# ThorLL/Element-Crush-Gym

Hardware: AMD Instinct MI355X
Metric: env-steps/sec (batched boards) at 1/2/4/8 MI355X, 9×9×6; bit-exact vs CPU (higher is better)
Workload: dtype int8; 1 GPU; C3: 1,048,576 boards per GPU, 9x9x6, Match3Env.step x 7466 (step kernel + overflow fixup + autoreset; N>1: RCCL reward/done all-gather once after the last step); boards_per_gpu=1048576, num_moves=20, env_goal=500, parallelism=dp1, hw_queues=8, autoreset=True

## Files before the change

### element-crush-gym_amd/csrc/m3_api.hip

```cpp
#include "m3_kernels.hpp"

#include <string>

namespace {
thread_local std::string g_err;
}

int set_err(int code, const char* fmt, ...) {
    char buf[512];
    va_list ap;
    va_start(ap, fmt);
    vsnprintf(buf, sizeof(buf), fmt, ap);
    va_end(ap);
    g_err = buf;
    return code;
}

#ifdef M3_SPLIT_TU
namespace m3k {
M3_INSTANTIATE(extern template, CF_0)
M3_INSTANTIATE(extern template, CF_1)
#ifndef M3_HEADLINE_ONLY
M3_INSTANTIATE(extern template, CF_2)
M3_INSTANTIATE(extern template, CF_3)
// ... 600 lines not shown
    return cnt[2] ? bad_cells_error() : M3_OK;
}

int m3_env_create(m3_ctx* c, int64_t n, int num_moves, int env_goal, m3_env** out) {
    CHECK_ARG(c && out && n > 0 && num_moves > 0, "bad arguments");
    CHECK_ARG(n < (int64_t)1 << 31, "n too large");
    int rc0 = check_ids_on_board(c);
    if (rc0) return rc0;
    *out = nullptr;
    HIP_TRY(hipSetDevice(c->device));
    m3_env* e = new m3_env;
    e->ctx = c;
    e->n = n;
    e->num_moves = num_moves;
    e->goal = env_goal;
    const size_t bytes = n * (size_t)c->N;
    hipError_t err = hipSuccess;
    auto alloc = [&](auto** p, size_t sz) {
        if (err == hipSuccess) err = hipMalloc((void**)p, sz ? sz : 4);
    };
    alloc(&e->boards[0], bytes);
    alloc(&e->boards[1], bytes);
    alloc(&e->seeds, n * 4);
    alloc(&e->flags, n * 4);
    alloc(&e->draws, n * 4);
    alloc(&e->legal, n * 4ull * c->AW);
    alloc(&e->score, n * 4);
    alloc(&e->moves, n * 4);
    alloc(&e->next_action, n * 4);
    alloc(&e->reward, n * 4);
    alloc(&e->done, n);
    alloc(&e->trunc, n);
    alloc(&e->counters, 64 * 4 * MAX_SHARDS);
    alloc(&e->ovf_list, n * 4);
    alloc(&e->packed, 2 * n * 4);
    alloc(&e->slot, n);
    alloc(&e->ne_words, (size_t)NSLOT * n * 4ull * ((c->N + 3) / 4));
    alloc(&e->ne_first, (size_t)NSLOT * n * 4);
    alloc(&e->ne_legal, (size_t)NSLOT * n * 4ull * c->AW);
    alloc(&e->ne_flags, (size_t)NSLOT * n * 4);
    alloc(&e->defer, n * 4);
    for (int p = 0; p < PF_LAG; ++p) {
        alloc(&e->pf_list[p], n * 4);
        alloc(&e->pf_seed[p], n * 4);
        alloc(&e->pf_slot[p], n * 4);
    }
    with_shape(c->shape, [&](auto cf) {
        using K = KS<decltype(cf)>;
        using St = LdsStore<decltype(cf), K::GCAP, K::B>;
        alloc(&e->spill, (size_t)MAX_SHARDS * K::SPILL_RECORDS * St::SPILL_WORDS * 4);
        alloc(&e->m397, (size_t)NSLOT * n * 4ull);
        constexpr size_t RW = CONT_REC<decltype(cf)>;
        if constexpr (K::CASCADE_LIMIT >= 0) alloc(&e->cont, RW * n * 4ull);
        if constexpr (RESET_TWO_STAGE<decltype(cf)>) alloc(&e->tab, (size_t)TwoStage<decltype(cf)>::TW * n * 4ull);
        if constexpr (RESET_TWO_STAGE_REJ<decltype(cf)>)
            alloc(&e->tab, (size_t)TwoStageRej<decltype(cf)>::TW * n * 4ull);
        return 0;
    });
    for (hipEvent_t& ev : e->gev)
        if (err == hipSuccess) err = hipEventCreateWithFlags(&ev, hipEventDisableTiming);
    {
        void* zp[] = {e->boards[0], e->boards[1], e->seeds, e->flags, e->draws, e->legal, e->score, e->moves,
                      e->next_action, e->reward, e->done, e->trunc, e->slot};
        size_t zb[] = {bytes, bytes, n * 4ull, n * 4ull, n * 4ull, n * 4ull * c->AW, n * 4ull, n * 4ull,
                       n * 4ull, n * 4ull, (size_t)n, (size_t)n, (size_t)n};
        for (int i = 0; i < 13 && err == hipSuccess; ++i) err = hipMemset(zp[i], 0, zb[i]);
    }
    if (err != hipSuccess) {
        m3_env_destroy(e);
        return set_err(M3_ERR_HIP, "env allocation (%lld boards): %s", (long long)n, hipGetErrorString(err));
    }
    int rc = m3_env_set_shards(e, 1);
    if (rc) {
        m3_env_destroy(e);
        return rc;
    }
    *out = e;
    return M3_OK;
}

int m3_env_set_shards(m3_env* e, int nshards) {
    CHECK_ARG(e && nshards >= 1 && nshards <= MAX_SHARDS, "nshards must be in [1, 8]");
    HIP_TRY(hipSetDevice(e->ctx->device));
    int rc = sync_env(e);
    if (rc) return rc;
    destroy_shards(e);
    const int64_t per = ((e->n + nshards - 1) / nshards + BLOCK - 1) / BLOCK * BLOCK;
    for (int s = 0; s < nshards; ++s) {
        m3_env::Shard sh;
        sh.off = std::min<int64_t>(e->n, s * per);
        sh.n = std::min<int64_t>(e->n, sh.off + per) - sh.off;
        if (M3_STREAM_PRIO) {
            int least = 0, greatest = 0;
            HIP_TRY(hipDeviceGetStreamPriorityRange(&least, &greatest));
            HIP_TRY(hipStreamCreateWithPriority(&sh.stream, hipStreamNonBlocking, greatest));
            HIP_TRY(hipStreamCreateWithPriority(&sh.pstream, hipStreamNonBlocking, least));
        } else {
            HIP_TRY(hipStreamCreateWithFlags(&sh.stream, hipStreamNonBlocking));
            HIP_TRY(hipStreamCreateWithFlags(&sh.pstream, hipStreamNonBlocking));
        }
        HIP_TRY(hipEventCreateWithFlags(&sh.ev, hipEventDisableTiming));
        for (hipEvent_t& ev : sh.pev) HIP_TRY(hipEventCreateWithFlags(&ev, hipEventDisableTiming));
        for (hipEvent_t& ev : sh.aev) HIP_TRY(hipEventCreateWithFlags(&ev, hipEventDisableTiming));
        e->shards.push_back(sh);
    }
    return M3_OK;
}

int m3_env_synchronize(m3_env* e) {
    CHECK_ARG(e, "null env");
    HIP_TRY(hipSetDevice(e->ctx->device));
    int rc = sync_env(e);
    if (rc) return rc;
    return ensure_fresh(e);
}

int m3_env_destroy(m3_env* e) {
    if (!e) return M3_OK;
    (void)hipSetDevice(e->ctx->device);
    (void)sync_env(e);
    destroy_shards(e);
    for (int p = 0; p < 2; ++p) {
        if (e->upload_ev[p]) (void)hipEventDestroy(e->upload_ev[p]);
        if (e->hstage[p]) (void)hipHostFree(e->hstage[p]);
    }
    if (e->ustream) (void)hipStreamDestroy(e->ustream);
    for (hipEvent_t ev : e->gev)
        if (ev) (void)hipEventDestroy(ev);
    void* ptrs[] = {e->boards[0], e->boards[1], e->seeds, e->flags, e->draws, e->legal, e->score, e->moves,
                    e->next_action, e->reward, e->done, e->trunc, e->actions[0], e->actions[1], e->counters,
                    e->ovf_list,
                    e->packed, e->gathered, e->slot, e->ne_words, e->ne_first, e->ne_legal, e->ne_flags,
                    e->spill, e->m397, e->cont, e->defer, e->tab};
    for (void* p : ptrs)
        if (p) (void)hipFree(p);
    for (int q = 0; q < PF_LAG; ++q)
        for (void* p : {(void*)e->pf_list[q], (void*)e->pf_seed[q], (void*)e->pf_slot[q]})
            if (p) (void)hipFree(p);
    if (e->comm) ncclCommDestroy(e->comm);
    for (hipEvent_t ev : e->tev) (void)hipEventDestroy(ev);
    delete e;
    return M3_OK;
}

int m3_env_reset(m3_env* e, const uint32_t* seeds, uint32_t seed_base) {
    CHECK_ARG(e, "null env");
    m3_ctx* c = e->ctx;
    HIP_TRY(hipSetDevice(c->device));
    int rc0 = sync_env(e);
    if (rc0) return rc0;
    if (seeds) {
        HIP_TRY(hipMemcpyAsync(e->seeds, seeds, e->n * 4, hipMemcpyHostToDevice, c->stream));
    } else {
        uint32_t* h = (uint32_t*)malloc(e->n * 4);
        if (!h) return set_err(M3_ERR_INVALID, "host allocation failed");
        for (int64_t i = 0; i < e->n; ++i) h[i] = seed_base + (uint32_t)i;
        hipError_t err = hipMemcpy(e->seeds, h, e->n * 4, hipMemcpyHostToDevice);
        free(h);
        HIP_TRY(err);
    }
    InitArgs a{};
    a.shape = c->sdesc;
    a.n = e->n;
    a.seeds = e->seeds;
    a.boards = e->boards[e->cur];
    a.first_action = e->next_action;
    a.legal = e->legal;
    a.score = e->score;
    a.moves = e->moves;
    a.reward = e->reward;
    a.done = e->done;
    a.trunc = e->trunc;
    a.flags = e->flags;
    a.draws = e->draws;
    a.m397 = e->m397;
    a.cstride = e->n;
    HIP_TRY(hipMemsetAsync(e->counters, 0, 64 * 4 * MAX_SHARDS, c->stream));
    HIP_TRY(hipMemsetAsync(e->slot, 0, e->n, c->stream));
    e->steps = 0;
    int rc = with_shape(c->shape, [&](auto cf) {
        int r = launch_init<decltype(cf)>(c->stream, a, e->n);
        if (r == M3_OK && e->autoreset) r = fill_next_slots<decltype(cf)>(e);
        return r;
    });
    if (rc) return rc;
    HIP_TRY(hipStreamSynchronize(c->stream));
// ... 338 lines not shown
```

### element-crush-gym_amd/csrc/m3_kernels.hpp

```cpp
#pragma once
#include <hip/hip_runtime.h>
#include <rccl/rccl.h>

#include <stdarg.h>
#include <stdio.h>
#include <string.h>

#include <algorithm>
#include <string>
#include <vector>

#include "../../include/m3.h"
#include "m3_rules.hpp"

using namespace m3;

int set_err(int code, const char* fmt, ...) __attribute__((format(printf, 2, 3)));

namespace {


#define HIP_TRY(expr)                                                                            \
    do {                                                                                         \
        hipError_t e_ = (expr);                                                                  \
        if (e_ != hipSuccess)                                                                    \
            return set_err(M3_ERR_HIP, "%s: %s (%s:%d)", #expr, hipGetErrorString(e_), __FILE__, \
                           __LINE__);                                                            \
    } while (0)

#define RCCL_TRY(expr)                                                                            \
    do {                                                                                          \
        ncclResult_t r_ = (expr);                                                                 \
        if (r_ != ncclSuccess) return set_err(M3_ERR_RCCL, "%s: %s", #expr, ncclGetErrorString(r_)); \
    } while (0)

#define CHECK_ARG(cond, msg)                                       \
    do {                                                           \
        if (!(cond)) return set_err(M3_ERR_INVALID, "%s", (msg)); \
    } while (0)

constexpr int BLOCK = 256;
constexpr int FIX_BLOCK = 64;
constexpr int FIX_GRID = 16;
constexpr int INIT_FIX_BLOCK = 64;
constexpr int INIT_BLOCK = 64;
#ifndef M3_WIDE_FRAME_LANES
#define M3_WIDE_FRAME_LANES 1
#endif
template <class CF>
constexpr uint32_t lanes_for() { return CF::W > 8 ? (uint32_t)M3_WIDE_FRAME_LANES : 64u; }
template <class CF>
constexpr bool INIT_INLINE_FIX = CF::N <= 128;
constexpr int MAX_SHARDS = 8;
#ifndef M3_RESET_KCAP
#define M3_RESET_KCAP 454
#endif
constexpr uint32_t RESET_KCAP = M3_RESET_KCAP;
#ifndef M3_PF_DIV
#define M3_PF_DIV 1
#endif
#ifndef M3_PF_DIV16
#define M3_PF_DIV16 2
#endif
#ifndef M3_COOP_GMAX
#define M3_COOP_GMAX 4096
#endif
#ifndef M3_PF_GRID
#define M3_PF_GRID 0
#endif
#ifndef M3_PF_COOP_GRID
#define M3_PF_COOP_GRID 0
#endif
#ifndef M3_RESET16_CHAIN2
#define M3_RESET16_CHAIN2 0
#endif
constexpr uint32_t RESET_ROUND_CAP = 1u << 14;

template <class CF>
struct KS {
    static constexpr int B = 64;
    static_assert(B == 64, "one-wave workgroups: lds_sync() orders a single wave's LDS accesses");
    static constexpr int GCAP = CF::N <= 128 ? 6 : 4;
    static constexpr int BPW = CF::W > 8 ? M3_WIDE_FRAME_LANES : B;
#ifndef M3_STEP_WPS
#define M3_STEP_WPS 4
#endif
#ifndef M3_STEP_WPS16
#define M3_STEP_WPS16 2
#endif
#ifndef M3_STEP_WPS_FRAME
#define M3_STEP_WPS_FRAME 1
#endif
    static constexpr int STEP_WPS = CF::DYN ? M3_STEP_WPS_FRAME : (CF::N > 128 ? M3_STEP_WPS16 : M3_STEP_WPS);
#ifndef M3_CONT_WPS
#define M3_CONT_WPS M3_STEP_WPS
#endif
    static constexpr int CONT_WPS = CF::N > 128 ? 1 : M3_CONT_WPS;
    static constexpr uint32_t SPILL_RECORDS = CF::W > 8 ? 256 : 4096;
    using Chain = std::conditional_t<(CF::N > 128), ChainMT1, ChainMT>;
    using Rng = Chain;
#ifndef M3_STEP_PRIO
#define M3_STEP_PRIO 0
#endif
#ifndef M3_STREAM_PRIO
#define M3_STREAM_PRIO 0
#endif
#ifndef M3_CASCADE_LIMIT
#define M3_CASCADE_LIMIT 2
#endif
#ifndef M3_CASCADE_LIMIT16
#define M3_CASCADE_LIMIT16 -1
#endif
    static constexpr int CASCADE_LIMIT = CF::N > 128 ? M3_CASCADE_LIMIT16 : M3_CASCADE_LIMIT;
};

#ifdef __HIP_DEVICE_COMPILE__
#define M3_LDS_AS __attribute__((address_space(3)))
#else
// ... 385 lines not shown
        ArrayStore<CF> st;
        apply_and_emit<CF>(P, a, b, mt, st, dm);
        planes_to_bytes<CF>(P, reinterpret_cast<uint8_t*>(a.out_boards + b * dm.cells()), dm);
    }
    if (a.clear_ovf) {
        __syncthreads();
        if (threadIdx.x == 0) *a.ovf_count = 0u;
    }
}

#ifndef M3_NSLOT
#define M3_NSLOT 4
#endif
constexpr int NSLOT = M3_NSLOT;
static_assert(NSLOT >= 2 && NSLOT <= 255, "slot index is a byte");
constexpr int PF_LAG = NSLOT - 1;
constexpr int CBLOCKS = PF_LAG + 1;
static_assert(8 * CBLOCKS <= 40, "the counter blocks end where a shard's stats begin (m3_env::counters, word 40)");
#ifndef M3_STAGE_PAD
#define M3_STAGE_PAD 1
#endif

}
namespace m3k {
struct InitArgs {
    Shape shape;
    int64_t n;
    const uint32_t* list;
    const uint32_t* list_seed;
    const uint32_t* list_slot;
    const uint32_t* list_count;
    const uint32_t* seeds;
    uint32_t seed_add;
    uint32_t slot0;
    const uint8_t* slot_of;
    int64_t sstride;
    int8_t* boards;
    uint32_t* board_words;
    uint32_t* draws;
    int32_t* first_action;
    uint32_t* legal;
    int32_t* score;
    int32_t* moves;
    int32_t* reward;
    uint8_t* done;
    uint8_t* trunc;
    uint32_t* flags;
    uint32_t* slot_flags;
    uint32_t* stats;
    uint32_t* m397;
    int64_t cstride;
    uint32_t* defer;
    uint32_t* defer_count;
    uint32_t* tab;
};
}
using m3k::InitArgs;
namespace {

__device__ __forceinline__ void init_item(const InitArgs& a, int64_t i, int64_t& b, uint32_t& seed, uint32_t& slot) {
    if (a.list) {
        b = (int64_t)a.list[i];
        seed = a.list_seed[i];
        slot = a.list_slot[i];
    } else {
        b = i;
        seed = a.seeds[b] + a.seed_add;
        slot = a.slot_of ? ((uint32_t)a.slot_of[b] + a.slot0) % (uint32_t)NSLOT : a.slot0;
    }
}

template <class CF>
__device__ __forceinline__ void init_store_board(const InitArgs& a, int64_t ob, const typename CF::Bd* P,
                                                 const typename CF::Dim& dm) {
    if constexpr (CF::DYN) {
        uint8_t* dst = a.board_words ? reinterpret_cast<uint8_t*>(a.board_words + ob * cell_words<CF>(dm))
                                     : reinterpret_cast<uint8_t*>(a.boards + ob * dm.cells());
        frame_to_bytes<CF>(P, dst, dm);
        return;
    }
    constexpr int NW = (CF::N + 3) / 4;
    uint32_t cw[NW];
    words_from_planes<CF>(P, cw);
    if (a.board_words) {
#pragma unroll
        for (int q = 0; q < NW; ++q) a.board_words[ob * NW + q] = cw[q];
    } else {
        store_cells<CF::N>(reinterpret_cast<uint8_t*>(a.boards + ob * CF::N), cw);
    }
}

template <class CF>
__device__ __forceinline__ void init_outputs(const InitArgs& a, int64_t b, int64_t ob, uint32_t seed, uint32_t m397,
                                             uint32_t draws, const typename CF::Bd* P,
                                             const typename CF::Dim& dm = typename CF::Dim{}) {
    typename CF::Bd HL, VL;
    legal_masks<CF>(P, special_mask<CF, CF::NP>(P), HL, VL, dm);
    uint32_t act[CF::AW];
    action_bits<CF>(HL, VL, act, dm);
    ChainMT rng;
    rng.init(seed, m397);
    const int fa = random_action<CF>(act, rng);
    if (a.draws) a.draws[ob] = draws;
    if (a.first_action) a.first_action[ob] = fa;
    if (a.legal) store_legal<CF>(a.legal + ob * dm.aw(), act, dm);
    if (a.score) a.score[b] = 0;
// ... 94 lines not shown
    uint32_t x = __builtin_amdgcn_readfirstlane(seed);
    for (int blk = 0; blk < 9; ++blk) {
        uint32_t col = 0u;
#pragma unroll
        for (int j = 0; j < 64; ++j) {
            asm volatile("v_writelane_b32 %0, %1, %2" : "+v"(col) : "s"(x), "n"(j));
            x = mt_init_next(x, (uint32_t)(blk * 64 + j) + 1u);
        }
        key[blk * 64 + lane] = col;
    }
    uint32_t col = 0u;
#pragma unroll
    for (int j = 0; j < 48; ++j) {
        asm volatile("v_writelane_b32 %0, %1, %2" : "+v"(col) : "s"(x), "n"(j));
        x = mt_init_next(x, (uint32_t)(576 + j) + 1u);
    }
    if (lane < 48) key[576 + lane] = col;
}

template <class CF>
__device__ uint32_t wave_reset(const InitArgs& a, int64_t item, uint32_t* key, uint8_t* cells, int lane) {
    int64_t b;
    uint32_t seed, slot;
    init_item(a, item, b, seed, slot);
    wave_init_key(key, seed, lane);
    wave_sync();
    const uint32_t m397 = key[397];
    uint32_t pos = 624u, k = 0u;
    typename CF::Bd P[CF::NP], mask;
    const int64_t ob = (int64_t)slot * a.sstride + b;
    constexpr int NW = (CF::N + 3) / 4;
    wave_fill<CF>(key, cells, lane, pos, k, nullptr);
    planes_from_words<CF>(reinterpret_cast<const uint32_t*>(cells), P);
    while (get_match_mask<CF>(P, mask)) {
        wave_fill<CF>(key, cells, lane, pos, k, &mask);
        planes_from_words<CF>(reinterpret_cast<const uint32_t*>(cells), P);
    }
    if (a.m397 && lane == 0) a.m397[(int64_t)slot * a.cstride + b] = m397;
    if (lane == 0) init_outputs<CF>(a, b, ob, seed, m397, k, P);
    if (a.board_words) {
        for (int q = lane; q < NW; q += 64)
            a.board_words[ob * NW + q] = reinterpret_cast<const uint32_t*>(cells)[q];
    } else {
        int8_t* dst = a.boards + ob * CF::N;
        for (int x = lane; x < CF::N; x += 64) dst[x] = (int8_t)cells[x];
    }
    wave_sync();
    return k;
}

template <class CF, bool REDO>
__global__ void __launch_bounds__(INIT_BLOCK) k_init(InitArgs a) {
    const int64_t cnt = a.list_count ? (int64_t)*a.list_count : a.n;
    if (a.stats && blockIdx.x == 0 && threadIdx.x == 0) atomicAdd(&a.stats[0], (uint32_t)cnt);
    __shared__ uint32_t tm_s[CF::BITS * TileGen<CF>::TWMAX * INIT_BLOCK];
    __shared__ uint32_t pos_s[TileGen<CF>::MAXR * INIT_BLOCK];
    uint32_t* tm = tm_s + threadIdx.x;
    uint32_t* pos = pos_s + threadIdx.x;
#ifdef M3_PHASE_PROF
    M3_PROF_LDS(INIT_BLOCK)
    Prof<NoStore> ps;
    ps.w = prof_s[threadIdx.x >> 6];
    const bool live = (int64_t)blockIdx.x * INIT_BLOCK < cnt;
    if (live) ps.begin();
#else
    NoStore* const pp = nullptr;
#endif
    static_assert(INIT_INLINE_FIX<CF> && INIT_BLOCK == 64, "the in-wave redo is one wave's");
    __shared__ uint32_t key_s[REDO ? 624 : 1];
    __shared__ __attribute__((aligned(16))) uint8_t cell_s[REDO ? (CF::N + 3) / 4 * 4 + 16 : 16];
    for (int64_t base = (int64_t)blockIdx.x * INIT_BLOCK; base < cnt; base += (int64_t)gridDim.x * INIT_BLOCK) {
        const int64_t i = base + threadIdx.x;
        bool ok = true;
        if (i < cnt) {
            int64_t b;
            uint32_t seed, slot;
            init_item(a, i, b, seed, slot);
            const uint32_t m397 = mt_state397(seed);
            const uint32_t kcap = a.defer ? RESET_KCAP : 624u;
#ifdef M3_PHASE_PROF
            ok = init_emit<CF>(a, b, seed, slot, m397, tm, pos, &ps, kcap);
#else
            ok = init_emit<CF>(a, b, seed, slot, m397, tm, pos, pp, kcap);
#endif
        }
        uint64_t bad = __ballot(!ok);
        if (!REDO) {
            if (bad) {
                const int lane = (int)threadIdx.x;
                uint32_t base = 0;
                if (lane == 0) base = atomicAdd(a.defer_count, (uint32_t)__popcll(bad));
                base = __shfl(base, 0);
                if (!ok) a.defer[base + (uint32_t)__popcll(bad & ((1ull << lane) - 1ull))] = (uint32_t)i;
            }
            continue;
        }
        if (bad && a.stats && threadIdx.x == 0) atomicAdd(&a.stats[1], (uint32_t)__builtin_popcountll(bad));
        if constexpr (REDO) {
            while (bad) {
                const int l = __builtin_ctzll(bad);
                bad &= bad - 1ull;
                wave_reset<CF>(a, __shfl(i, l), key_s, cell_s, (int)threadIdx.x);
            }
        }
    }
#ifdef M3_PHASE_PROF
    if (live) ps.end(1);
#endif
}

template <class CF>
__global__ void __launch_bounds__(64) k_init_coop(InitArgs a) {
    __shared__ uint32_t key_s[624];
    __shared__ __attribute__((aligned(16))) uint8_t cell_s[(CF::N + 3) / 4 * 4 + 16];
    const uint32_t cnt = *a.defer_count;
    const int lane = (int)threadIdx.x;
    for (uint32_t q = blockIdx.x; q < cnt; q += gridDim.x) {
        wave_reset<CF>(a, a.defer[q], key_s, cell_s, lane);
        if (a.stats && lane == 0) atomicAdd(&a.stats[1], 1u);
    }
}

template <class R, class = void>
struct HasBulk : std::false_type {};
template <class R>
struct HasBulk<R, std::void_t<decltype(std::declval<R&>().bulk_ready(1u))>> : std::true_type {};

template <class CF, class RNG>
__device__ __forceinline__ void fill_round(typename CF::Bd* P, RNG& mt, const typename CF::Bd* only) {
#pragma unroll
    for (int w = 0; w < CF::W; ++w) {
        constexpr int BITS = CF::BITS;
        const int nbits = CF::N - 32 * w < 32 ? CF::N - 32 * w : 32;
        uint32_t t[BITS];
#pragma unroll
        for (int p = 0; p < BITS; ++p) t[p] = 0u;
        int bit = 0;
        if constexpr (CF::TILE_RNG != 0u && CF::TILE_RNG == CF::TILE_MASK && HasBulk<RNG>::value) {
            if (mt.bulk_ready((uint32_t)nbits)) {
#pragma unroll
                for (int j = 0; j < nbits; ++j) {
                    const uint32_t v = (mt.bulk_out((uint32_t)j) & CF::TILE_MASK) + 1u;
#pragma unroll
                    for (int p = 0; p < BITS; ++p) t[p] |= ((v >> p) & 1u) << j;
                }
                mt.bulk_skip((uint32_t)nbits);
                bit = nbits;
            }
        }
        for (; bit < nbits; ++bit) {
            uint32_t v = 1u;
            if constexpr (CF::TILE_RNG != 0u) {
                do {
                    v = mt.next32() & CF::TILE_MASK;
                } while (v > CF::TILE_RNG);
                v += 1u;
            }
#pragma unroll
            for (int p = 0; p < BITS; ++p) t[p] |= ((v >> p) & 1u) << bit;
        }
        const uint32_t m = only ? only->w[w] : 0xFFFFFFFFu;
#pragma unroll
        for (int p = 0; p < BITS; ++p) P[p].w[w] = (P[p].w[w] & ~m) | (t[p] & m);
    }
}
// ... 385 lines not shown
        lds_to_planes<CF>(lds, t, P, dm);
        legal_masks<CF>(P, special_mask<CF, CF::NP>(P), HL, VL, dm);
        uint32_t act[CF::AW];
        action_bits<CF>(HL, VL, act, dm);
        store_legal<CF>(legal + (b0 + t) * dm.aw(), act, dm);
    }
}


}
namespace m3k {
struct EnvArgs {
    Shape shape;
    int64_t n;
    int num_moves, goal;
    int autoreset;
    uint32_t stride;
    const int8_t* cur;
    int8_t* nxt;
    const int32_t* actions;
    uint32_t* seeds;
    int32_t* score;
    int32_t* moves;
    int32_t* next_action;
    int32_t* reward;
    uint8_t* done;
    uint8_t* trunc;
    uint32_t* flags;
    uint32_t* draws;
    uint32_t* legal;
    int32_t* packed;
    uint32_t* counters;
    uint32_t* spill;
    uint32_t* stats;
    uint32_t* ovf_list;
    uint8_t* slot;
    const uint32_t* ne_words;
    const int32_t* ne_first;
    const uint32_t* ne_legal;
    const uint32_t* ne_flags;
    uint32_t* pf_list;
    uint32_t* pf_seed;
    uint32_t* pf_slot;
    const uint32_t* m397;
    int64_t cstride;
    uint32_t* cont;
    int64_t cont_stride;
    uint32_t* zero_next;
};
}
using m3k::EnvArgs;
namespace {

enum : int { CNT_OVF = 0, CNT_PF_DEFER = 2, CNT_SPILL = 3, CNT_CONT = 4, CNT_PF = 5 };

template <class CF>
struct EnvFin {
    static constexpr bool CELLS_IN_REGS = !CF::DYN;
    static constexpr int NWS = (CF::N + 3) / 4;
    uint32_t ndraws, f, nflags, s_old, seed;
    int r, tr, dn, sc, mv1, na, first;
    bool reset;
    int64_t ob;
    uint32_t act[CF::AW];
    uint32_t lg[CF::AW];
    uint32_t cw[CELLS_IN_REGS ? NWS : 1];
};

template <class CF, class RNG, class Store>
__device__ __forceinline__ bool env_fin_begin(typename CF::Bd* P, const EnvArgs& a, int64_t b, RNG& rng, Store& st,
                                              int r, uint32_t f, const typename CF::Bd& HL, const typename CF::Bd& VL,
                                              int mv, int sc0, const typename CF::Dim& dm, uint8_t* row,
                                              EnvFin<CF>& e, const uint32_t* known_slot = nullptr,
                                              const uint32_t* known_seed = nullptr, bool cells = true) {
    const bool stepped = !(f & (FLAG_TERMINAL | FLAG_BAD_ACTION));
    e.r = r;
    e.sc = sc0 + r;
    e.mv1 = mv + 1;
    e.tr = e.sc >= a.goal;
    e.dn = e.tr || e.mv1 == a.num_moves;
    e.ndraws = stepped ? rng.draws() : 0u;
    action_bits<CF>(HL, VL, e.act, dm);
    e.na = -1;
    if (stepped) {
        e.na = random_action<CF>(e.act, rng);
        if (rng.overflow) return false;
        if (e.na < 0) f |= FLAG_NO_LEGAL;
    }
    e.f = f;
    mark<PH_NEXT>(st);
    e.reset = e.dn && a.autoreset;
    if (row) planes_to_bytes<CF>(P, row, dm);
    mark<PH_TBYTES>(st);
    const int AW = dm.aw();
    e.s_old = 0u;
    e.seed = 0u;
    e.ob = 0;
    e.first = -1;
    e.nflags = 0u;
    if (e.reset) {
        const uint32_t s_old = known_slot ? *known_slot : a.slot[b];
        e.seed = (known_seed ? *known_seed : a.seeds[b]) + a.stride;
        const uint32_t s_new = s_old + 1u == (uint32_t)NSLOT ? 0u : s_old + 1u;
        e.ob = (int64_t)s_new * a.cstride + b;
        e.first = a.ne_first[e.ob];
        e.nflags = a.ne_flags ? a.ne_flags[e.ob] : 0u;
        if (a.legal) {
// ... 18 lines not shown
                                              const EnvFin<CF>& e, const typename CF::Dim& dm, uint8_t* row,
                                              bool cells = true) {
    const int AW = dm.aw();
    a.draws[b] = e.ndraws;
    a.reward[b] = e.r;
    a.trunc[b] = (uint8_t)e.tr;
    a.done[b] = (uint8_t)e.dn;
    a.flags[b] = e.f | e.nflags;
    if (a.packed) a.packed[b] = (e.r << 2) | (e.tr << 1) | e.dn;
    if (!e.reset) {
        a.score[b] = e.sc;
        a.moves[b] = e.mv1;
        a.next_action[b] = e.na;
        if (a.legal) store_legal<CF>(a.legal + b * AW, e.act, dm);
    } else {
        a.slot[b] = (uint8_t)e.s_old;
        a.seeds[b] = e.seed;
        a.score[b] = 0;
        a.moves[b] = 0;
        a.next_action[b] = e.first;
        if (a.legal) {
#pragma unroll
            for (int i = 0; i < CF::AW; ++i)
                if (i < AW) a.legal[b * AW + i] = e.lg[i];
        }
        if constexpr (EnvFin<CF>::CELLS_IN_REGS) {
            if (!cells) {
            } else if (row) {
                store_cells<CF::N>(row, e.cw);
            } else {
                planes_from_words<CF>(e.cw, P);
            }
        } else {
            const uint8_t* src = reinterpret_cast<const uint8_t*>(a.ne_words + e.ob * cell_words<CF>(dm));
            if (row) {
                for (int x = 0; x < dm.cells(); ++x) row[x] = src[x];
            } else {
                frame_from_bytes<CF>(src, P, dm);
            }
        }
    }
    mark<PH_RESET>(st);
}

__device__ __forceinline__ void env_fin_queue(const EnvArgs& a, int64_t b, uint32_t q, uint32_t seed, uint32_t s_new) {
    a.pf_list[q] = (uint32_t)b;
    a.pf_seed[q] = seed + (uint32_t)(NSLOT - 1) * a.stride;
    a.pf_slot[q] = s_new == 0u ? (uint32_t)(NSLOT - 1) : s_new - 1u;
}

#ifndef M3_COOP_CELLS
#define M3_COOP_CELLS 1
#endif
template <class CF>
__device__ __forceinline__ void coop_reset_cells(const EnvArgs& a, uint64_t m, int64_t ob, uint8_t* lds, int row_stride) {
    constexpr int NWS = EnvFin<CF>::NWS;
    static_assert(NWS <= 64, "one word per lane per board");
    constexpr int PER = 64 / NWS;
    constexpr int BATCH = PER >= 3 ? 1 : 4;
    const int lane = (int)__lane_id(), j = lane / NWS, w = lane - j * NWS;
    while (m) {
        uint32_t v[BATCH];
        int src[BATCH];
#pragma unroll
        for (int u = 0; u < BATCH; ++u) {
            src[u] = -1;
#pragma unroll
            for (int k = 0; k < PER; ++k) {
                const int l = m ? __ffsll((unsigned long long)m) - 1 : -1;
                if (k == j) src[u] = l;
                if (m) m &= m - 1ull;
            }
            const int64_t sob = __shfl(ob, src[u] < 0 ? 0 : src[u]);
            v[u] = (j < PER && src[u] >= 0) ? a.ne_words[sob * NWS + w] : 0u;
        }
#pragma unroll
        for (int u = 0; u < BATCH; ++u) {
            if (j < PER && src[u] >= 0) {
                uint8_t* dst = lds + src[u] * row_stride + 4 * w;
                if constexpr (CF::N % 4 == 0) {
                    *reinterpret_cast<uint32_t*>(dst) = v[u];
                } else {
#pragma unroll
                    for (int y = 0; y < 4; ++y)
                        if (4 * w + y < CF::N) dst[y] = (uint8_t)(v[u] >> (8 * y));
                }
            }
        }
    }
}

struct FinOpts {
    const uint32_t* slot = nullptr;
    const uint32_t* seed = nullptr;
    bool cells = true;
    bool* reset = nullptr;
    int64_t* ob = nullptr;
};

__device__ __forceinline__ uint32_t lane_rank(uint64_t m) {
    return (uint32_t)__popcll(m & ((1ull << __lane_id()) - 1ull));
}

template <class CF, class RNG, class Store>
__device__ __forceinline__ bool env_finish(typename CF::Bd* P, const EnvArgs& a, int64_t b, RNG& rng, Store& st,
                                           int r, uint32_t f, const typename CF::Bd& HL, const typename CF::Bd& VL,
                                           int mv, int sc0, const typename CF::Dim& dm, uint8_t* row = nullptr,
                                           FinOpts o = FinOpts{}) {
    EnvFin<CF> e;
    if (!env_fin_begin<CF>(P, a, b, rng, st, r, f, HL, VL, mv, sc0, dm, row, e, o.slot, o.seed, o.cells)) return false;
    if (o.reset) *o.reset = e.reset;
    if (o.ob) *o.ob = e.ob;
// ... 415 lines not shown
#undef X
    if (r < 3 || c < 3 || r > MAX_FRAME || c > MAX_FRAME || t < 2 || t > 31) return -1;
    return N_SPECIALISED + (frame_side(r, c) == 32 ? 4 : 0) + bits_for_types(t) - 2;
}

}

struct m3_ctx {
    int device = 0;
    int R = 0, C = 0, T = 0, N = 0, A = 0, AW = 0;
    int shape = -1;
    Shape sdesc{};
    hipStream_t stream = nullptr;
    void* dbuf = nullptr;
    size_t dcap = 0;
    void* hbuf = nullptr;
    void* hdev = nullptr;
    size_t hcap = 0;
    uint32_t* counters = nullptr;
};

struct m3_env {
    m3_ctx* ctx = nullptr;
    int64_t n = 0;
    int num_moves = 20, goal = 500;
    int autoreset = 0;
    uint32_t stride = 0;
    bool ready = false;
    uint32_t loaded = 0;
    bool legal_eager = false;
    bool stale = false;
    int8_t* boards[2] = {nullptr, nullptr};
    int cur = 0;
    uint32_t *seeds = nullptr, *flags = nullptr, *draws = nullptr, *legal = nullptr;
    int32_t *score = nullptr, *moves = nullptr, *next_action = nullptr, *reward = nullptr;
    uint8_t *done = nullptr, *trunc = nullptr;
    int32_t* actions[2] = {nullptr, nullptr};
    int32_t* hstage[2] = {nullptr, nullptr};
    hipStream_t ustream = nullptr;
    hipEvent_t upload_ev[2] = {nullptr, nullptr};
    bool upload_pend[2] = {false, false};
    bool upload_this = false;
    uint32_t* counters = nullptr;
    uint32_t* ovf_list = nullptr;
    uint32_t* spill = nullptr;
    uint8_t* slot = nullptr;
    uint32_t* ne_words = nullptr;
    int32_t* ne_first = nullptr;
    uint32_t* ne_legal = nullptr;
    uint32_t* ne_flags = nullptr;
    uint32_t* m397 = nullptr;
    uint32_t* cont = nullptr;
    uint32_t* defer = nullptr;
    uint32_t* tab = nullptr;
    uint32_t *pf_list[PF_LAG] = {}, *pf_seed[PF_LAG] = {}, *pf_slot[PF_LAG] = {};
    int64_t steps = 0;
    int32_t* packed = nullptr;
    int32_t* gathered = nullptr;
    ncclComm_t comm = nullptr;
    int nranks = 1, rank = 0;
    std::vector<hipEvent_t> tev;
    int tcap = 0, tn = 0;
    struct Shard {
        int64_t off = 0, n = 0;
        hipStream_t stream = nullptr, pstream = nullptr;
        hipEvent_t ev = nullptr;
        hipEvent_t aev[2] = {};
        bool apending[2] = {};
        hipEvent_t pev[PF_LAG] = {};
        bool ppending[PF_LAG] = {};
    };
    std::vector<Shard> shards;
    hipEvent_t gev[2] = {nullptr, nullptr};
    bool gpend[2] = {false, false};
};

using CF_0 = Cfg<9, 9, 6>;
using CF_1 = Cfg<16, 16, 8>;
using CF_2 = FCfg<2>;
using CF_3 = FCfg<3>;
using CF_4 = FCfg<4>;
using CF_5 = FCfg<5>;
using CF_6 = FCfg<2, 32>;
using CF_7 = FCfg<3, 32>;
using CF_8 = FCfg<4, 32>;
using CF_9 = FCfg<5, 32>;
constexpr int N_CONFIGS = 10;

namespace m3k {

template <class CF>
int fix_grid() { return (int)(FIX_GRID * 64 / lanes_for<CF>()); }

template <class CF>
int grid_for(int64_t n) { return (int)((n + KS<CF>::BPW - 1) / KS<CF>::BPW); }

template <class CF>
int launch_apply(m3_ctx* c, const ApplyArgs& a) {
    if (a.n == 0) return M3_OK;
    hipLaunchKernelGGL(k_apply<CF>, dim3(grid_for<CF>(a.n)), dim3(KS<CF>::B), 0, c->stream, a);
    HIP_TRY(hipGetLastError());
    hipLaunchKernelGGL(k_apply_fix<CF>, dim3(a.clear_ovf ? 1 : fix_grid<CF>()), dim3(FIX_BLOCK), 0, c->stream, a);
    HIP_TRY(hipGetLastError());
    return M3_OK;
}

template <class CF>
int launch_init(hipStream_t stream, const InitArgs& a, int64_t max_items) {
    if (max_items == 0) return M3_OK;
    int64_t g = (max_items + INIT_BLOCK - 1) / INIT_BLOCK;
    if (g > 4096) g = 4096;
    const int64_t pf_cap = a.defer ? (int64_t)M3_PF_GRID : 0, coop_cap = a.defer ? (int64_t)M3_PF_COOP_GRID : 0;
    if (pf_cap > 0 && g > pf_cap) g = pf_cap;
    if constexpr (INIT_INLINE_FIX<CF>) {
        if constexpr (RESET_TWO_STAGE_REJ<CF>) {
            if (a.tab && a.defer) {
                int64_t ga = (max_items + TwoStageRej<CF>::G - 1) / TwoStageRej<CF>::G;
                ga = ga > 2048 ? 2048 : ga;
                hipLaunchKernelGGL(k_reset_stream_rej<CF>, dim3((unsigned)ga), dim3(64), 0, stream, a);
                HIP_TRY(hipGetLastError());
                hipLaunchKernelGGL(k_reset_tiles_rej<CF>, dim3((unsigned)g), dim3(64), 0, stream, a);
                HIP_TRY(hipGetLastError());
                int64_t gc = max_items / 64 + 1;
                gc = gc < 64 ? 64 : (gc > 4096 ? 4096 : gc);
                if (coop_cap > 0 && gc > coop_cap) gc = coop_cap;
                hipLaunchKernelGGL(k_init_coop<CF>, dim3((unsigned)gc), dim3(64), 0, stream, a);
                HIP_TRY(hipGetLastError());
                return M3_OK;
            }
        }
        if (a.defer) hipLaunchKernelGGL((k_init<CF, false>), dim3((unsigned)g), dim3(INIT_BLOCK), 0, stream, a);
        else hipLaunchKernelGGL((k_init<CF, true>), dim3((unsigned)g), dim3(INIT_BLOCK), 0, stream, a);
        if (a.defer) {
            HIP_TRY(hipGetLastError());
            int64_t gc = max_items / 16 + 1;
            gc = gc < 64 ? 64 : (gc > M3_COOP_GMAX ? M3_COOP_GMAX : gc);
            if (coop_cap > 0 && gc > coop_cap) gc = coop_cap;
            hipLaunchKernelGGL(k_init_coop<CF>, dim3((unsigned)gc), dim3(64), 0, stream, a);
        }
    } else if constexpr (!CF::DYN && M3_RESET16_CHAIN2) {
        hipLaunchKernelGGL(k_init_chain2<CF>, dim3((unsigned)g), dim3(INIT_BLOCK), 0, stream, a);
        if (a.defer) {
            HIP_TRY(hipGetLastError());
            int64_t gc = max_items / 32 + 1;
            gc = gc < 64 ? 64 : (gc > 4096 ? 4096 : gc);
            hipLaunchKernelGGL(k_init_coop<CF>, dim3((unsigned)gc), dim3(64), 0, stream, a);
        }
    } else if (RESET_TWO_STAGE<CF> && a.tab && a.defer) {
        if constexpr (RESET_TWO_STAGE<CF>) {
            const InitArgs& s = a;
            int64_t ga = (max_items + TwoStage<CF>::G - 1) / TwoStage<CF>::G;
            ga = ga > 2048 ? 2048 : ga;
            if (pf_cap > 0 && ga > pf_cap) ga = pf_cap;
            hipLaunchKernelGGL(k_reset_stream<CF>, dim3((unsigned)ga), dim3(64), 0, stream, s);
            HIP_TRY(hipGetLastError());
            hipLaunchKernelGGL(k_reset_tiles<CF>, dim3((unsigned)(g > 4096 ? 4096 : g)), dim3(64), 0, stream, s);
            HIP_TRY(hipGetLastError());
            int64_t gc = max_items / 32 + 1;
            gc = gc < 64 ? 64 : (gc > M3_COOP_GMAX ? M3_COOP_GMAX : gc);
            if (coop_cap > 0 && gc > coop_cap) gc = coop_cap;
            hipLaunchKernelGGL(k_init_coop<CF>, dim3((unsigned)gc), dim3(64), 0, stream, a);
        }
    } else {
        const int64_t gl = (max_items + lanes_for<CF>() - 1) / lanes_for<CF>();
        hipLaunchKernelGGL(k_init_fix_lane<CF>, dim3((unsigned)(gl > 4096 ? 4096 : gl)), dim3(INIT_FIX_BLOCK), 0,
                           stream, a);
    }
    HIP_TRY(hipGetLastError());
    return M3_OK;
}

template <class CF>
int launch_legal(m3_ctx* c, int64_t n, const int8_t* boards, uint32_t* legal) {
    if (n == 0) return M3_OK;
    hipLaunchKernelGGL(k_legal<CF>, dim3(grid_for<CF>(n)), dim3(KS<CF>::B), 0, c->stream, c->sdesc, n, boards, legal);
    HIP_TRY(hipGetLastError());
    return M3_OK;
}

template <class CF>
void prefetch_args(const m3_env* e, int64_t o, InitArgs& r) {
    r.shape = e->ctx->sdesc;
    r.sstride = e->n;
    r.board_words = e->ne_words + o * ((e->ctx->N + 3) / 4);
    r.first_action = e->ne_first + o;
    r.legal = e->ne_legal + o * e->ctx->AW;
    r.m397 = e->m397 + o;
    r.slot_flags = e->ne_flags + o;
    r.cstride = e->n;
    if constexpr (RESET_TWO_STAGE<CF>) r.tab = e->tab ? e->tab + o * TwoStage<CF>::TW : nullptr;
    if constexpr (RESET_TWO_STAGE_REJ<CF>) r.tab = e->tab ? e->tab + o * TwoStageRej<CF>::TW : nullptr;
// ... 37 lines not shown
    a.draws = e->draws + o;
    a.legal = e->legal_eager ? e->legal + o * AW : nullptr;
    a.packed = e->comm ? e->packed + (size_t)pb * e->n + o : nullptr;
    a.counters = cnt;
    a.spill = e->spill + (size_t)s * KS<CF>::SPILL_RECORDS * LdsStore<CF, KS<CF>::GCAP, KS<CF>::B>::SPILL_WORDS;
    a.stats = base + 40;
    a.ovf_list = e->ovf_list + o;
    a.slot = e->slot + o;
    a.ne_words = e->ne_words + o * ((N + 3) / 4);
    a.ne_first = e->ne_first + o;
    a.ne_legal = e->ne_legal + o * AW;
    a.ne_flags = e->ne_flags + o;
    a.pf_list = e->pf_list[par] + o;
    a.pf_seed = e->pf_seed[par] + o;
    a.pf_slot = e->pf_slot[par] + o;
    a.m397 = e->m397 + o;
    a.cstride = e->n;
    a.cont = KS<CF>::CASCADE_LIMIT >= 0 ? e->cont + o * CONT_REC<CF> : nullptr;
    a.cont_stride = CONT_REC<CF>;
    a.zero_next = base + 8 * ((e->steps + 1) % CBLOCKS);
    const bool timed = e->tn < e->tcap;
    if (timed) HIP_TRY(hipEventRecord(e->tev[3 * e->tn], st));
    hipLaunchKernelGGL(k_env_step<CF>, dim3(grid_for<CF>(sh.n)), dim3(KS<CF>::B), 0, st, a);
    HIP_TRY(hipGetLastError());
    if (timed) HIP_TRY(hipEventRecord(e->tev[3 * e->tn + 1], st));
    if constexpr (KS<CF>::CASCADE_LIMIT >= 0) {
        const int64_t g = ((int64_t)(sh.n * 0.25) + KS<CF>::B - 1) / KS<CF>::B;
        hipLaunchKernelGGL(k_env_cont_grid<CF>, dim3((unsigned)(g > 0 ? g : 1)), dim3(KS<CF>::B), 0, st, a);
        HIP_TRY(hipGetLastError());
    }
    hipLaunchKernelGGL(k_env_fix<CF>, dim3(env_fix_lanes<CF>() == 1u ? 64 : fix_grid<CF>()), dim3(FIX_BLOCK), 0, st, a);
    HIP_TRY(hipGetLastError());
    if (timed) {
        HIP_TRY(hipEventRecord(e->tev[3 * e->tn + 2], st));
        e->tn++;
    }
    HIP_TRY(hipEventRecord(sh.ev, st));
    if (e->upload_this) {
        HIP_TRY(hipEventRecord(sh.aev[pb], st));
        sh.apending[pb] = true;
    }
    if (e->autoreset) {
        HIP_TRY(hipStreamWaitEvent(sh.pstream, sh.ev, 0));
        InitArgs r{};
        r.n = sh.n;
        r.list = e->pf_list[par] + o;
        r.list_seed = e->pf_seed[par] + o;
        r.list_slot = e->pf_slot[par] + o;
        r.list_count = &cnt[CNT_PF];
        r.stats = base + 41;
        if constexpr (INIT_INLINE_FIX<CF> || (!CF::DYN && M3_RESET16_CHAIN2) || RESET_TWO_STAGE<CF>) {
            r.defer = e->defer + o;
            r.defer_count = &cnt[CNT_PF_DEFER];
        }
        prefetch_args<CF>(e, o, r);
#ifndef M3_DEBUG_NO_PREFETCH
        constexpr int64_t PF_DIV = CF::DYN ? 8 : (CF::N > 128 ? M3_PF_DIV16 : M3_PF_DIV);
        int rc = launch_init<CF>(sh.pstream, r, sh.n / PF_DIV + 1);
        if (rc) return rc;
#endif
        HIP_TRY(hipEventRecord(sh.pev[par], sh.pstream));
        sh.ppending[par] = true;
    }
    return M3_OK;
}

template <class CF>
int launch_env_step(m3_env* e, const int32_t* d_actions) {
    for (int s = 0; s < (int)e->shards.size(); ++s) {
        int rc = launch_env_shard<CF>(e, s, d_actions);
        if (rc) return rc;
    }
    e->upload_this = false;
    e->gpend[e->steps & 1] = false;
    e->cur ^= 1;
    e->steps++;
    return M3_OK;
}

template <class CF>
int fill_next_slots(m3_env* e) {
    m3_ctx* c = e->ctx;
    for (uint32_t k = 1; k < (uint32_t)NSLOT; ++k) {
        InitArgs r{};
        r.n = e->n;
        r.seeds = e->seeds;
        r.seed_add = k * e->stride;
        r.slot0 = k;
        r.slot_of = e->slot;
        prefetch_args<CF>(e, 0, r);
        int rc = launch_init<CF>(c->stream, r, e->n);
        if (rc) return rc;
    }
    HIP_TRY(hipStreamSynchronize(c->stream));
    return M3_OK;
}

template <class CF>
int rederive(m3_env* e) {
    m3_ctx* c = e->ctx;
    HIP_TRY(hipMemsetAsync(e->counters, 0, 64 * 4 * MAX_SHARDS, c->stream));
    HIP_TRY(hipMemsetAsync(e->slot, 0, e->n, c->stream));
    const int64_t g = std::min<int64_t>((e->n + 255) / 256, 4096);
    hipLaunchKernelGGL(k_mt397, dim3((unsigned)g), dim3(256), 0, c->stream, e->n, e->seeds, e->m397);
    HIP_TRY(hipGetLastError());
    int rc = launch_legal<CF>(c, e->n, e->boards[e->cur], e->legal);
// ... 32 lines not shown
```

Baseline: 2.668 billion env-steps/s.

## Add dense retry stage between inline reset and cooperative reset, plus early exits

```diff
diff --git a/element-crush-gym_amd/csrc/m3_api.hip b/element-crush-gym_amd/csrc/m3_api.hip
--- a/element-crush-gym_amd/csrc/m3_api.hip
+++ b/element-crush-gym_amd/csrc/m3_api.hip
@@ -676,6 +676,7 @@
         alloc(&e->m397, (size_t)NSLOT * n * 4ull);
         constexpr size_t RW = CONT_REC<decltype(cf)>;
         if constexpr (K::CASCADE_LIMIT >= 0) alloc(&e->cont, RW * n * 4ull);
+        if constexpr (INIT_INLINE_FIX<decltype(cf)>) alloc(&e->defer2, n * 4ull);
         if constexpr (RESET_TWO_STAGE<decltype(cf)>) alloc(&e->tab, (size_t)TwoStage<decltype(cf)>::TW * n * 4ull);
         if constexpr (RESET_TWO_STAGE_REJ<decltype(cf)>)
             alloc(&e->tab, (size_t)TwoStageRej<decltype(cf)>::TW * n * 4ull);
@@ -755,7 +756,7 @@
                     e->next_action, e->reward, e->done, e->trunc, e->actions[0], e->actions[1], e->counters,
                     e->ovf_list,
                     e->packed, e->gathered, e->slot, e->ne_words, e->ne_first, e->ne_legal, e->ne_flags,
-                    e->spill, e->m397, e->cont, e->defer, e->tab};
+                    e->spill, e->m397, e->cont, e->defer, e->defer2, e->tab};
     for (void* p : ptrs)
         if (p) (void)hipFree(p);
     for (int q = 0; q < PF_LAG; ++q)
diff --git a/element-crush-gym_amd/csrc/m3_kernels.hpp b/element-crush-gym_amd/csrc/m3_kernels.hpp
--- a/element-crush-gym_amd/csrc/m3_kernels.hpp
+++ b/element-crush-gym_amd/csrc/m3_kernels.hpp
@@ -64,6 +64,18 @@
 #endif
 #ifndef M3_COOP_GMAX
 #define M3_COOP_GMAX 4096
+#endif
+#ifndef M3_RESET_EARLY_EXIT
+#define M3_RESET_EARLY_EXIT 1
+#endif
+#ifndef M3_DENSE_MIN
+#define M3_DENSE_MIN 4096
+#endif
+#ifndef M3_DENSE_PRIO
+#define M3_DENSE_PRIO 3
+#endif
+#ifndef M3_DENSE_GMAX
+#define M3_DENSE_GMAX 1024
 #endif
 #ifndef M3_PF_GRID
 #define M3_PF_GRID 0
@@ -555,6 +567,8 @@
     int64_t cstride;
     uint32_t* defer;
     uint32_t* defer_count;
+    uint32_t* defer2;
+    uint32_t* defer2_count;
     uint32_t* tab;
 };
 }
@@ -755,6 +769,9 @@
 template <class CF, bool REDO>
 __global__ void __launch_bounds__(INIT_BLOCK) k_init(InitArgs a) {
     const int64_t cnt = a.list_count ? (int64_t)*a.list_count : a.n;
+    if constexpr (!REDO && M3_RESET_EARLY_EXIT) {
+        if ((int64_t)blockIdx.x * INIT_BLOCK >= cnt) return;
+    }
     if (a.stats && blockIdx.x == 0 && threadIdx.x == 0) atomicAdd(&a.stats[0], (uint32_t)cnt);
     __shared__ uint32_t tm_s[CF::BITS * TileGen<CF>::TWMAX * INIT_BLOCK];
     __shared__ uint32_t pos_s[TileGen<CF>::MAXR * INIT_BLOCK];
@@ -813,7 +830,50 @@
 }
 
 template <class CF>
+__global__ void __launch_bounds__(INIT_BLOCK) k_init_dense(InitArgs a) {
+    const uint32_t cnt = *a.defer_count;
+    if (blockIdx.x * (uint32_t)INIT_BLOCK >= cnt) return;
+    if (a.stats && blockIdx.x == 0 && threadIdx.x == 0) atomicAdd(&a.stats[1], cnt);
+    if (cnt <= (uint32_t)M3_DENSE_MIN) {
+        if (blockIdx.x == 0) {
+            for (uint32_t q = threadIdx.x; q < cnt; q += INIT_BLOCK) a.defer2[q] = a.defer[q];
+            if (threadIdx.x == 0) *a.defer2_count = cnt;
+        }
+        return;
+    }
+    if constexpr (M3_DENSE_PRIO > 0) __builtin_amdgcn_s_setprio(M3_DENSE_PRIO);
+    __shared__ uint32_t tm_s[CF::BITS * TileGen<CF>::TWMAX * INIT_BLOCK];
+    __shared__ uint32_t pos_s[TileGen<CF>::MAXR * INIT_BLOCK];
+    uint32_t* tm = tm_s + threadIdx.x;
+    uint32_t* pos = pos_s + threadIdx.x;
+    static_assert(INIT_INLINE_FIX<CF> && INIT_BLOCK == 64, "one wave per block: the ballot is the block's");
+    const int lane = (int)threadIdx.x;
+    for (uint32_t base = blockIdx.x * (uint32_t)INIT_BLOCK; base < cnt; base += gridDim.x * (uint32_t)INIT_BLOCK) {
+        const uint32_t q = base + (uint32_t)lane;
+        bool ok = true;
+        uint32_t item = 0u;
+        if (q < cnt) {
+            item = a.defer[q];
+            int64_t b;
+            uint32_t seed, slot;
+            init_item(a, (int64_t)item, b, seed, slot);
+            ok = init_emit<CF>(a, b, seed, slot, mt_state397(seed), tm, pos, (NoStore*)nullptr, 624u);
+        }
+        const uint64_t bad = __ballot(!ok);
+        if (bad) {
+            uint32_t at = 0;
+            if (lane == 0) at = atomicAdd(a.defer2_count, (uint32_t)__popcll(bad));
+            at = __shfl(at, 0);
+            if (!ok) a.defer2[at + (uint32_t)__popcll(bad & ((1ull << lane) - 1ull))] = item;
+        }
+    }
+}
+
+template <class CF>
 __global__ void __launch_bounds__(64) k_init_coop(InitArgs a) {
+    if constexpr (INIT_INLINE_FIX<CF> && M3_RESET_EARLY_EXIT) {
+        if (blockIdx.x >= *a.defer_count) return;
+    }
     __shared__ uint32_t key_s[624];
     __shared__ __attribute__((aligned(16))) uint8_t cell_s[(CF::N + 3) / 4 * 4 + 16];
     const uint32_t cnt = *a.defer_count;
@@ -1305,7 +1365,7 @@
 using m3k::EnvArgs;
 namespace {
 
-enum : int { CNT_OVF = 0, CNT_PF_DEFER = 2, CNT_SPILL = 3, CNT_CONT = 4, CNT_PF = 5 };
+enum : int { CNT_OVF = 0, CNT_PF_DEFER = 2, CNT_SPILL = 3, CNT_CONT = 4, CNT_PF = 5, CNT_PF_DEFER2 = 6 };
 
 template <class CF>
 struct EnvFin {
@@ -1430,12 +1490,15 @@
 #ifndef M3_COOP_CELLS
 #define M3_COOP_CELLS 1
 #endif
+#ifndef M3_COOP_BATCH9
+#define M3_COOP_BATCH9 1
+#endif
 template <class CF>
 __device__ __forceinline__ void coop_reset_cells(const EnvArgs& a, uint64_t m, int64_t ob, uint8_t* lds, int row_stride) {
     constexpr int NWS = EnvFin<CF>::NWS;
     static_assert(NWS <= 64, "one word per lane per board");
     constexpr int PER = 64 / NWS;
-    constexpr int BATCH = PER >= 3 ? 1 : 4;
+    constexpr int BATCH = PER >= 3 ? M3_COOP_BATCH9 : 4;
     const int lane = (int)__lane_id(), j = lane / NWS, w = lane - j * NWS;
     while (m) {
         uint32_t v[BATCH];
@@ -1957,6 +2020,7 @@
     uint32_t* m397 = nullptr;
     uint32_t* cont = nullptr;
     uint32_t* defer = nullptr;
+    uint32_t* defer2 = nullptr;
     uint32_t* tab = nullptr;
     uint32_t *pf_list[PF_LAG] = {}, *pf_seed[PF_LAG] = {}, *pf_slot[PF_LAG] = {};
     int64_t steps = 0;
@@ -2038,10 +2102,18 @@
         else hipLaunchKernelGGL((k_init<CF, true>), dim3((unsigned)g), dim3(INIT_BLOCK), 0, stream, a);
         if (a.defer) {
             HIP_TRY(hipGetLastError());
+            int64_t gd = max_items / (16 * INIT_BLOCK) + 1;
+            gd = gd > M3_DENSE_GMAX ? M3_DENSE_GMAX : gd;
+            hipLaunchKernelGGL(k_init_dense<CF>, dim3((unsigned)gd), dim3(INIT_BLOCK), 0, stream, a);
+            HIP_TRY(hipGetLastError());
+            InitArgs c = a;
+            c.defer = a.defer2;
+            c.defer_count = a.defer2_count;
+            c.stats = nullptr;
             int64_t gc = max_items / 16 + 1;
             gc = gc < 64 ? 64 : (gc > M3_COOP_GMAX ? M3_COOP_GMAX : gc);
             if (coop_cap > 0 && gc > coop_cap) gc = coop_cap;
-            hipLaunchKernelGGL(k_init_coop<CF>, dim3((unsigned)gc), dim3(64), 0, stream, a);
+            hipLaunchKernelGGL(k_init_coop<CF>, dim3((unsigned)gc), dim3(64), 0, stream, c);
         }
     } else if constexpr (!CF::DYN && M3_RESET16_CHAIN2) {
         hipLaunchKernelGGL(k_init_chain2<CF>, dim3((unsigned)g), dim3(INIT_BLOCK), 0, stream, a);
@@ -2185,6 +2257,10 @@
         if constexpr (INIT_INLINE_FIX<CF> || (!CF::DYN && M3_RESET16_CHAIN2) || RESET_TWO_STAGE<CF>) {
             r.defer = e->defer + o;
             r.defer_count = &cnt[CNT_PF_DEFER];
+            if constexpr (INIT_INLINE_FIX<CF>) {
+                r.defer2 = e->defer2 + o;
+                r.defer2_count = &cnt[CNT_PF_DEFER2];
+            }
         }
         prefetch_args<CF>(e, o, r);
 #ifndef M3_DEBUG_NO_PREFETCH
```

After: 2.681 billion env-steps/s, median of 3. About the same (+0.5%).
